# SHI-Labs/Self-Similarity-Grouping

Hardware: AMD Instinct MI355X
Metric: images/s embed + s/iter for NxN rerank+DBSCAN, N=16k, 1/2/4/8 GPU (higher is better)
Workload: dtype f32 (embed: split-half operands hi+lo on fp16 MFMA, fp32 accumulate, 6e-8 max error vs the fp32 reference features) / exact int64 via int8 MFMA digits + f64 + f16 (distance, re-rank: half semantics, bit-exact)

## Files before the change

### include/ssg_hip.h

```cpp
#ifndef SSG_HIP_H
#define SSG_HIP_H

#include <stddef.h>
#include <stdint.h>

#ifdef __cplusplus
extern "C" {
#endif

typedef struct ihipStream_t* ssg_stream_t;

#define SSG_OK 0
#define SSG_ERR_INVALID (-1)
#define SSG_ERR_HIP (-2)
#define SSG_ERR_OVERFLOW (-3)
#define SSG_ERR_NAN (-4)

const char* ssg_last_error(void);
int ssg_version(void);
uint16_t ssg_double_to_half_bits(double d);

int ssg_range_stats_f32(const float* a, int rows_a, const float* b, int rows_b, int d, float* out4, ssg_stream_t stream);
int ssg_row_norms_f64(const float* x, int n, int d, int round_to_half, double* norms, ssg_stream_t stream);
int ssg_sqdist_self_f16(const float* x, const double* norms, int N, int d, int row0, int nrows, int memory_save, uint16_t* D, uint32_t* rowmax,
// ... 106 lines not shown
int ssg_conv1x1_dual_nhwc_x(const void* in, const void* in2, const void* w, const float* bias, void* out, int B, int H, int W, int Cin,
                            int H2, int W2, int Cin2, int stride2, int Cout, int relu, int flags, float acc_scale, const float* ch_scale,
                            int32_t* overflow, ssg_stream_t stream);
#define SSG_CONV_W_TILED 4
int ssg_conv_weights_tile_supported(int Cout, int Kpad);
int ssg_conv_weights_tile(const void* w, int Cout, int Kpad, void* wt, ssg_stream_t stream);
int ssg_conv2d_nhwc_xt(const void* in, const void* w, const void* wt, const float* bias, const void* res, void* out, int B, int H, int W, int Cin,
                       int Cout, int KH, int KW, int stride, int pad, int relu, int flags, float acc_scale, const float* ch_scale,
                       int32_t* overflow, ssg_stream_t stream);
int ssg_conv1x1_dual_nhwc_xt(const void* in, const void* in2, const void* w, const void* wt, const float* bias, void* out, int B, int H, int W, int Cin,
                             int H2, int W2, int Cin2, int stride2, int Cout, int relu, int flags, float acc_scale, const float* ch_scale,
                             int32_t* overflow, ssg_stream_t stream);
int ssg_conv_pair_supported(int K1, int C, int N2);
int ssg_conv_pair_nhwc_x(const void* y2, const void* w3, const float* b3, const float* cs3, const void* res, void* out,
                         const void* w1n, const float* b1n, const float* cs1n, void* y1n, int M, int K1, int C, int N2,
                         int32_t* overflow, ssg_stream_t stream);
int ssg_bottleneck_supported(int H, int W, int CIN, int C, int MID);
int ssg_bottleneck_nhwc_x(const void* x, const void* w1, const float* b1, const float* cs1, const void* w2, const float* b2, const float* cs2,
                          const void* w3, const float* b3, const float* cs3, void* out, int B, int H, int W, int C, int MID,
                          int32_t* overflow, ssg_stream_t stream);
int ssg_bottleneck_ds_nhwc_x(const void* x, const void* w1, const float* b1, const float* cs1, const void* w2, const float* b2, const float* cs2,
                             const void* w3cat, const float* b3, const float* cs3, void* out, int B, int H, int W, int CIN, int C, int MID,
                             int32_t* overflow, ssg_stream_t stream);
int ssg_basicblock_supported(int H, int W, int C);
int ssg_basicblock_nhwc_x(const void* x, const void* w1, const float* b1, const float* cs1, const void* w2, const float* b2, const float* cs2,
                          void* out, int B, int H, int W, int C, int32_t* overflow, ssg_stream_t stream);
int ssg_stem_pool_supported(int H, int W);
int ssg_stem_pool_nchw_x(const float* images, int flip, const void* w, const float* bias, const float* ch_scale, void* out, int B, int H, int W,
                         int32_t* overflow, ssg_stream_t stream);
int ssg_nchw_to_nhwc4_h4l4(const float* in, void* out, int B, int H, int W, int flip, ssg_stream_t stream);
int ssg_maxpool3x3s2_h8l8(const void* in, void* out, int B, int H, int W, int C, ssg_stream_t stream);
int ssg_gap_stripes_h8l8(const void* in, float* out, int B, int H, int W, int C, int num_split, ssg_stream_t stream);
int ssg_h8l8_encode(const float* in, void* out, int64_t n, float scale, ssg_stream_t stream);
int ssg_h8l8_decode(const void* in, float* out, int64_t n, float scale, ssg_stream_t stream);
int ssg_pairwise_sqdist_f32(const float* x, const float* y, int m, int n, int d, int self_form, float* ws, float* out, ssg_stream_t stream);
int ssg_nchw_to_nhwc4(const float* in, float* out, int B, int H, int W, int flip, ssg_stream_t stream);
int ssg_maxpool3x3s2_nhwc(const float* in, float* out, int B, int H, int W, int C, ssg_stream_t stream);
int ssg_gap_stripes(const float* in, float* out, int B, int H, int W, int C, int num_split, ssg_stream_t stream);
int ssg_flip_sum_l2norm(const float* a, const float* b, float* out, int rows, int C, ssg_stream_t stream);

int ssg_knn_sets(const uint16_t* D, const int32_t* rank, int N, int row0, int nrows, int K, int cap, int32_t* a_idx, uint16_t* a_val,
                 int32_t* a_nnz, int32_t* overflow, ssg_stream_t stream);
int ssg_set_jaccard_rows(const int32_t* a_idx, const int32_t* a_nnz, int capA, const int64_t* colptr, const int32_t* inv_row, int N, int row0,
                         int nrows, uint16_t one_minus_lambda_half, uint16_t* Jp, ssg_stream_t stream);

int ssg_seqdist_f64(const float* x, int m, const float* y, int n, int d, int take_sqrt, double* out, int64_t ld, ssg_stream_t stream);
// ... 192 lines not shown
```

### self-similarity-grouping_amd/csrc/bottleneck.hip

```cpp
#include "ssg_common.h"
#include <cstdlib>

#ifndef SSG_BN_NT_STORE
#define SSG_BN_NT_STORE 1
#endif
#ifndef SSG_BN_NT_RES
#define SSG_BN_NT_RES 1
#endif

namespace ssg {
namespace bneck {

typedef float v16f __attribute__((ext_vector_type(16)));
typedef unsigned int v4u __attribute__((ext_vector_type(4)));
typedef _Float16 v8h __attribute__((ext_vector_type(8)));
typedef float v4f __attribute__((ext_vector_type(4)));

struct Params {
  const float* x; float* out;
  const float* w1; const float* b1; const float* cs1;
  const float* w2; const float* b2; const float* cs2;
  const float* w3; const float* b3; const float* cs3;
  int B, H;
  int* overflow;
  unsigned long long* prof = nullptr;
};
#ifdef SSG_BN_PROF
#define SSG_BN_STAMP(I_) { if (p.prof && threadIdx.x == 0) p.prof[(size_t)blockIdx.x * 8 + (I_)] = __builtin_readcyclecounter(); }
#else
#define SSG_BN_STAMP(I_)
#endif

constexpr int cmax(int a, int b) { return a > b ? a : b; }

template <int C, int MID, int IW, int TH, int CIN = C, int NW = 4>
struct Cfg {
  static constexpr int HROWS = TH + 2, NPIX1 = HROWS * IW, NPIX = TH * IW;
  static constexpr int NTHR = NW * 64, RPP = NTHR / 4;
#ifndef SSG_BN_K1T
#define SSG_BN_K1T 32
#endif
#ifndef SSG_BN_K1T4
#define SSG_BN_K1T4 32
#endif
  static constexpr int K1T = NW == 8 ? SSG_BN_K1T : SSG_BN_K1T4, KS1 = K1T / 16, CPR1 = 4 * KS1, RPP1 = NTHR / CPR1;
  static constexpr int XROWS = (NPIX1 + RPP1 - 1) / RPP1 * RPP1;
  static constexpr int P1 = 80;
  static constexpr int P1T = K1T * 4 + 16;
// ... 25 lines not shown
  return (unsigned)__builtin_bit_cast(unsigned short, a) | ((unsigned)__builtin_bit_cast(unsigned short, b) << 16);
}
__device__ __forceinline__ void encode4(const float4 v, uint2& hi, uint2& lo) {
  const _Float16 h0 = (_Float16)v.x, h1 = (_Float16)v.y, h2 = (_Float16)v.z, h3 = (_Float16)v.w;
  hi = make_uint2(pack2(h0, h1), pack2(h2, h3));
  lo = make_uint2(pack2((_Float16)(v.x - (float)h0), (_Float16)(v.y - (float)h1)), pack2((_Float16)(v.z - (float)h2), (_Float16)(v.w - (float)h3)));
}
__device__ __forceinline__ unsigned hi_nonfinite_bits(const uint2 hi) {
  return ((hi.x & 0x7c007c00u) + 0x04000400u) | ((hi.y & 0x7c007c00u) + 0x04000400u);
}
__device__ __forceinline__ float hlo(unsigned u) { return (float)__builtin_bit_cast(_Float16, (unsigned short)(u & 0xffffu)); }
__device__ __forceinline__ float hhi(unsigned u) { return (float)__builtin_bit_cast(_Float16, (unsigned short)(u >> 16)); }
__device__ __forceinline__ float4 decode4(const uint2 hi, const uint2 lo) {
  return make_float4(hlo(hi.x) + hlo(lo.x), hhi(hi.x) + hhi(lo.x), hlo(hi.y) + hlo(lo.y), hhi(hi.y) + hhi(lo.y));
}
__device__ __forceinline__ float4 relu4(float4 v) {
  return make_float4(v.x > 0.f ? v.x : 0.f, v.y > 0.f ? v.y : 0.f, v.z > 0.f ? v.z : 0.f, v.w > 0.f ? v.w : 0.f);
}

__device__ __forceinline__ void bn_dma16(const __amdgpu_buffer_rsrc_t r, unsigned lds_addr, unsigned voff, int soff) {
  __builtin_amdgcn_raw_ptr_buffer_load_lds(r, (__attribute__((address_space(3))) void*)(uintptr_t)lds_addr, 16, voff, soff, 0, 0);
}

template <int C, int MID, int IW, int TH, int CIN, int NW>
__global__ __launch_bounds__(NW * 64, NW == 4 ? 2 : 1) void bottleneck_kernel(Params p) {
  using K = Cfg<C, MID, IW, TH, CIN, NW>;
  constexpr bool DS = K::DS;
  extern __shared__ __attribute__((aligned(16))) unsigned char smem[];
  const int tid = (int)threadIdx.x, lane = tid & 63, wave = tid >> 6, l32 = lane & 31, h = lane >> 5;
  const int tiles_img = p.H / TH, ntiles = p.B * tiles_img;
  int T;
  {
    const int b = (int)blockIdx.x, q = ntiles / 8, r = ntiles % 8, x = b % 8, s = b / 8;
    T = (x < r ? x * (q + 1) : r * (q + 1) + (x - r) * q) + s;
  }
  const int img = T / tiles_img, ty0 = (T - img * tiles_img) * TH;
  SSG_BN_STAMP(0)
  if (K::ZERO_EARLY && tid < K::PY / 16) *reinterpret_cast<uint4*>(smem + K::ZERO_OFF + tid * 16) = make_uint4(0u, 0u, 0u, 0u);

  constexpr int RPP = K::RPP, RPP1 = K::RPP1, AU = K::XROWS / RPP1, WU = MID / RPP1;
  const int ck = tid & 3, r0 = tid >> 2;
  const int ck1 = tid % K::CPR1, r1 = tid / K::CPR1;
  const float* ximg = p.x + (int64_t)img * p.H * IW * CIN;
  const __amdgpu_buffer_rsrc_t xrsrc = __builtin_amdgcn_make_buffer_rsrc(const_cast<float*>(ximg), 0, (unsigned)(p.H * IW * CIN * 4), 0x00020000);
  constexpr int MT1 = K::NPIX1 / 32, NT1 = MID / 32;
  constexpr int WC1 = NT1 < NW / 2 ? NT1 : NW / 2, WR1 = NW / WC1, MTW1 = (MT1 + WR1 - 1) / WR1, NTW1 = NT1 / WC1;
  static_assert(NT1 % WC1 == 0 && (WR1 * MTW1) * 32 <= K::XROWS, "phase-1 tiles divide over the waves");
// ... 177 lines not shown
        v = relu4(v);
        if (!inside) v = make_float4(0.f, 0.f, 0.f, 0.f);
        uint2 hi, lo;
        encode4(v, hi, lo);
        ovf |= hi_nonfinite_bits(hi);
        unsigned char* d = smem + (hp0 + l32) * K::PY + (ch >> 3) * 32 + h * 8;
        *reinterpret_cast<uint2*>(d) = hi; *reinterpret_cast<uint2*>(d + 16) = lo;
      }
  }
  if (!K::ZERO_EARLY && tid < K::PY / 16) *reinterpret_cast<uint4*>(smem + K::ZERO_OFF + tid * 16) = make_uint4(0u, 0u, 0u, 0u);
  SSG_BN_STORE2(0, 0)
  __syncthreads();
  SSG_BN_STAMP(2)

  constexpr int WC2 = NW / 4, NT2 = MID / 32 / WC2;
  const int pt2 = wave / WC2, cb2 = (wave % WC2) * NT2;
  v16f acc2[NT2];
#pragma unroll
  for (int j = 0; j < NT2; j++)
#pragma unroll
    for (int r = 0; r < 16; r++) acc2[j][r] = 0.f;
  const int m2 = pt2 * 32 + l32, ty2 = m2 / IW, tx2 = m2 - ty2 * IW;
  float4 cs2r[NT2][4], b2r[NT2][4];
#pragma unroll
  for (int j = 0; j < NT2; j++)
#pragma unroll
    for (int q = 0; q < 4; q++) {
      cs2r[j][q] = *reinterpret_cast<const float4*>(p.cs2 + (cb2 + j) * 32 + 8 * q + 4 * h); b2r[j][q] = *reinterpret_cast<const float4*>(p.b2 + (cb2 + j) * 32 + 8 * q + 4 * h);
    }
#define SSG_BN_STEP2(KT_, S_, B_)                                                                                     \
  {                                                                                                                  \
    if ((KT_) + K::PD2 < K::NK2) SSG_BN_LOAD2((KT_) + K::PD2, S_)                                                     \
    _Pragma("unroll") for (int sub = 0; sub < K::KT2; sub++) {                                                       \
      const int kt_ = (KT_) * K::KT2 + sub;                                                                          \
      const int chunk = kt_ / 9, tap = kt_ - chunk * 9, r = tap / 3, s = tap - r * 3;                                \
      const int xin = tx2 + s - 1;                                                                                   \
      const int abase = (xin >= 0 && xin < IW) ? ((ty2 + r) * IW + xin) * K::PY : K::ZERO_OFF;                       \
      const unsigned char* wb = smem + K::W2_OFF + (B_) * K::BUF2 + (cb2 * 32 + l32) * K::P2 + sub * 128 + h * 32;     \
      v8h xh_[2], xl_[2], wh_[2][NT2], wl_[2][NT2];                                                                  \
      _Pragma("unroll") for (int ks = 0; ks < 2; ks++) {                                                             \
        const unsigned char* q_ = smem + abase + (chunk * 4 + ks * 2 + h) * 32;                                      \
        xh_[ks] = *reinterpret_cast<const v8h*>(q_); xl_[ks] = *reinterpret_cast<const v8h*>(q_ + 16);               \
        _Pragma("unroll") for (int j = 0; j < NT2; j++) {                                                            \
          wh_[ks][j] = *reinterpret_cast<const v8h*>(wb + j * 32 * K::P2 + ks * 64);                                 \
          wl_[ks][j] = *reinterpret_cast<const v8h*>(wb + j * 32 * K::P2 + ks * 64 + 16); }                          \
      }                                                                                                              \
      _Pragma("unroll") for (int ks = 0; ks < 2; ks++) {                                                             \
        _Pragma("unroll") for (int j = 0; j < NT2; j++) acc2[j] = __builtin_amdgcn_mfma_f32_32x32x16_f16(wh_[ks][j], xl_[ks], acc2[j], 0, 0, 0); \
        _Pragma("unroll") for (int j = 0; j < NT2; j++) acc2[j] = __builtin_amdgcn_mfma_f32_32x32x16_f16(wl_[ks][j], xh_[ks], acc2[j], 0, 0, 0); \
        _Pragma("unroll") for (int j = 0; j < NT2; j++) acc2[j] = __builtin_amdgcn_mfma_f32_32x32x16_f16(wh_[ks][j], xh_[ks], acc2[j], 0, 0, 0); \
      }                                                                                                              \
    }                                                                                                                \
    if ((KT_) + 1 < K::NK2) SSG_BN_STORE2((B_) ^ 1, ((S_) + 1) % K::PD2)                                              \
    __syncthreads();                                                                                                 \
  }
  static_assert(K::NK2 % 6 == 0 && 6 % K::PD2 == 0, "phase-2 ring");
#pragma unroll
  for (int kt0 = 0; kt0 < K::NK2; kt0 += 6) {
    SSG_BN_STEP2(kt0, 0 % K::PD2, 0) SSG_BN_STEP2(kt0 + 1, 1 % K::PD2, 1) SSG_BN_STEP2(kt0 + 2, 2 % K::PD2, 0)
    SSG_BN_STEP2(kt0 + 3, 3 % K::PD2, 1) SSG_BN_STEP2(kt0 + 4, 4 % K::PD2, 0) SSG_BN_STEP2(kt0 + 5, 5 % K::PD2, 1)
  }
#undef SSG_BN_STEP2
  SSG_BN_STAMP(3)
#undef SSG_BN_LOAD2
#undef SSG_BN_STORE2

  constexpr int CU3 = C / RPP;
  constexpr int K3 = MID + (DS ? CIN : 0);
  const float* w3p = p.w3 + (int64_t)r0 * K3 + ck * 4;
  v4f sc3[2][CU3];
#define SSG_BN_LOAD3(T_, S_)                                                                                         \
  { _Pragma("unroll") for (int u = 0; u < CU3; u++) sc3[S_][u] = *reinterpret_cast<const v4f*>(w3p + (int64_t)(RPP * u) * K3 + (T_) * 16); }
#define SSG_BN_STORE3(BUF_, S_)                                                                                      \
  { unsigned char* sb_ = smem + K::W3_OFF + (BUF_) * K::BUF3;                                                        \
    _Pragma("unroll") for (int u = 0; u < CU3; u++) *reinterpret_cast<v4f*>(sb_ + (r0 + RPP * u) * K::P1 + ck * 16) = sc3[S_][u]; }
  SSG_BN_LOAD3(0, 0)
  SSG_BN_LOAD3(1, 1)
  constexpr int WC3 = NW / 4, NT3 = C / 32 / WC3;
  const int pt3 = wave / WC3, cb3 = (wave % WC3) * NT3;
  const int64_t gpix0 = ((int64_t)img * p.H + ty0) * IW + pt3 * 32;
  constexpr int NXK = DS ? CIN / 16 : 1;
  v8h xrh[NXK], xrl[NXK];
  if constexpr (DS) {
    const float* xq = p.x + (gpix0 + l32) * CIN + h * 8;
#pragma unroll
    for (int t = 0; t < NXK; t++) { xrh[t] = *reinterpret_cast<const v8h*>(xq + t * 16); xrl[t] = *reinterpret_cast<const v8h*>(xq + t * 16 + 4); }
  }
  unsigned char* myrows = smem + (pt3 * 32) * K::PY;
#pragma unroll
// ... 108 lines not shown
      const float4 rw = rr[j & 1][it];
      float4 r4;
      {
        const unsigned a0 = __float_as_uint(rw.x), a1 = __float_as_uint(rw.y), a2 = __float_as_uint(rw.z), a3 = __float_as_uint(rw.w);
        const unsigned g0 = lane_xor1((odd ? a0 : a2)), g1 = lane_xor1((odd ? a1 : a3));
        const unsigned h0 = odd ? g0 : a0, h1 = odd ? g1 : a1, l0 = odd ? a2 : g0, l1 = odd ? a3 : g1;
        r4 = decode4(make_uint2(h0, h1), make_uint2(l0, l1));
      }
      v.x += r4.x; v.y += r4.y; v.z += r4.z; v.w += r4.w;
      }
      v = relu4(v);
      uint2 hp, lp;
      encode4(v, hp, lp);
      ovf |= hi_nonfinite_bits(hp);
      const unsigned rx = lane_xor1((odd ? hp.x : lp.x)), ry = lane_xor1((odd ? hp.y : lp.y));
      const uint4 stv = make_uint4(odd ? rx : hp.x, odd ? ry : hp.y, odd ? lp.x : rx, odd ? lp.y : ry);
#if SSG_BN_NT_STORE
      { const v4u sv_ = {stv.x, stv.y, stv.z, stv.w}; __builtin_nontemporal_store(sv_, reinterpret_cast<v4u*>(outp + (int64_t)pr * C + col)); }
#else
      *reinterpret_cast<uint4*>(outp + (int64_t)pr * C + col) = stv;
#endif
    }
    __builtin_amdgcn_fence(__ATOMIC_ACQ_REL, "wavefront");
  }
  if ((ovf & 0x80008000u) && p.overflow) *p.overflow = 1;
  SSG_BN_STAMP(5)
}

template <int C, int MID, int IW, int TH>
struct CfgH {
  static constexpr int NW = 4, NTHR = NW * 64, HROWS = TH + 2, NPIX1 = HROWS * IW, NPIX = TH * IW;
  static constexpr int MH = MID / 2;
  static constexpr int K1T = 32, P1T = K1T * 4, CPR1 = 8, RPP1 = NTHR / CPR1;
  static constexpr int XROWS = NPIX1, BUF1 = (XROWS + MID) * P1T;
  static constexpr int NK1 = C / K1T, PD1 = 2;
  static constexpr int PYH = MH * 4 + 16;
  static constexpr int ZERO_OFF = NPIX1 * PYH;
  static constexpr int P2 = 144, W2_OFF = (ZERO_OFF + PYH + 255) / 256 * 256, BUF2 = MID * P2;
  static constexpr int NK2H = (MH / 32) * 9, PD2 = 3;
  static constexpr int NCP = 128, NPASS = C / NCP, KT3 = MID / 32;
  static constexpr int EP = 36, PATCH = 32 * EP * 4;
  static constexpr int LDS = cmax(2 * BUF1, W2_OFF + 2 * BUF2);
  static_assert(NPIX == 128 && NPIX1 % RPP1 == 0 && MID % RPP1 == 0 && MH == 64 && MID == NCP && NK1 % PD1 == 0 && NK2H % 6 == 0 && KT3 == 4, "layer2 shape");
  static_assert(((NPIX1 + 31) / 32 + 1) / 2 == 3 && 6 * 32 <= XROWS + MID, "phase 1: 2 x 3 pixel tiles, the sixth one reads W1 rows of the stage");
  static_assert(RPP1 % 16 == 0 && XROWS % 16 == 0, "the swizzle of a row is that of its thread (r1) / its lane (l32)");
  static_assert(NW * PATCH <= ZERO_OFF && 32 * P2 == PATCH, "patches live in the dead y1 rows");
// ... 293 lines not shown
#else
        *reinterpret_cast<uint4*>(outp + (int64_t)pr * C + col) = stv;
#endif
      }
      __builtin_amdgcn_fence(__ATOMIC_ACQ_REL, "wavefront");
    }
  }
#undef SSG_BH_RESLOAD
#undef SSG_BH_STORE3
#undef SSG_BH_LOAD3
  if ((ovf & 0x80008000u) && p.overflow) *p.overflow = 1;
  SSG_BN_STAMP(5)
}

}
}

extern "C" int ssg_bottleneck_supported(int H, int W, int CIN, int C, int MID) {
  if (C == 256 && MID == 64 && (CIN == 256 || CIN == 64) && W == 32 && H > 0 && H % 4 == 0) return 1;
  if (C == 512 && MID == 128 && CIN == 512 && W == 16 && H > 0 && H % 8 == 0) return 1;
  return 0;
}

template <int C, int MID, int IW, int TH, int CIN, int NW>
static int launch_bottleneck(const ssg::bneck::Params& p, hipStream_t stream) {
  using namespace ssg::bneck;
  using K = Cfg<C, MID, IW, TH, CIN, NW>;
  static bool attr_set = false;
  if (!attr_set) {
    SSG_HIP(hipFuncSetAttribute((const void*)bottleneck_kernel<C, MID, IW, TH, CIN, NW>, hipFuncAttributeMaxDynamicSharedMemorySize, K::LDS));
    attr_set = true;
  }
  hipLaunchKernelGGL((bottleneck_kernel<C, MID, IW, TH, CIN, NW>), dim3(p.B * (p.H / TH)), dim3(NW * 64), K::LDS, stream, p);
  SSG_LAUNCH_CHECK("bottleneck_kernel");
  return SSG_OK;
}

template <int C, int MID, int IW, int TH>
static int launch_bottleneck_halves(const ssg::bneck::Params& p, hipStream_t stream) {
  using namespace ssg::bneck;
  using K = CfgH<C, MID, IW, TH>;
  static bool attr_set = false;
  if (!attr_set) {
    SSG_HIP(hipFuncSetAttribute((const void*)bottleneck_halves_kernel<C, MID, IW, TH>, hipFuncAttributeMaxDynamicSharedMemorySize, K::LDS));
    attr_set = true;
  }
  hipLaunchKernelGGL((bottleneck_halves_kernel<C, MID, IW, TH>), dim3(p.B * (p.H / TH)), dim3(K::NTHR), K::LDS, stream, p);
  SSG_LAUNCH_CHECK("bottleneck_halves_kernel");
  return SSG_OK;
}

#ifndef SSG_BN_L2_WAVES_DEFAULT
#define SSG_BN_L2_WAVES_DEFAULT 4
#endif

extern "C" int ssg_bottleneck_nhwc_x(const void* x, const void* w1, const float* b1, const float* cs1, const void* w2, const float* b2, const float* cs2,
                                     const void* w3, const float* b3, const float* cs3, void* out, int B, int H, int W, int C, int MID,
                                     int32_t* overflow, hipStream_t stream) {
  using namespace ssg::bneck;
  if (B <= 0 || !ssg_bottleneck_supported(H, W, C, C, MID) || !cs1 || !cs2 || !cs3 || x == out) {
    ssg_set_error("ssg_bottleneck_nhwc_x: unsupported block B=%d H=%d W=%d C=%d MID=%d (see ssg_bottleneck_supported)", B, H, W, C, MID);
    return SSG_ERR_INVALID;
  }
  Params p;
  p.x = (const float*)x; p.out = (float*)out;
  p.w1 = (const float*)w1; p.b1 = b1; p.cs1 = cs1; p.w2 = (const float*)w2; p.b2 = b2; p.cs2 = cs2; p.w3 = (const float*)w3; p.b3 = b3; p.cs3 = cs3;
  p.B = B; p.H = H; p.overflow = overflow;
  if (C == 512) {
    const char* e = getenv("SSG_BN_L2_WAVES");
    const int nw = e && *e ? atoi(e) : SSG_BN_L2_WAVES_DEFAULT;
    if (nw == 4) return launch_bottleneck_halves<512, 128, 16, 8>(p, stream);
    if (nw == 8) return launch_bottleneck<512, 128, 16, 8, 512, 8>(p, stream);
    ssg_set_error("ssg_bottleneck_nhwc_x: SSG_BN_L2_WAVES=%s (4 or 8)", e);
    return SSG_ERR_INVALID;
  }
  return launch_bottleneck<256, 64, 32, 4, 256, 4>(p, stream);
}

extern "C" int ssg_bottleneck_ds_nhwc_x(const void* x, const void* w1, const float* b1, const float* cs1, const void* w2, const float* b2, const float* cs2,
                                        const void* w3cat, const float* b3, const float* cs3, void* out, int B, int H, int W, int CIN, int C, int MID,
                                        int32_t* overflow, hipStream_t stream) {
  using namespace ssg::bneck;
  if (B <= 0 || CIN == C || !ssg_bottleneck_supported(H, W, CIN, C, MID) || !cs1 || !cs2 || !cs3) {
    ssg_set_error("ssg_bottleneck_ds_nhwc_x: unsupported block B=%d H=%d W=%d CIN=%d C=%d MID=%d (see ssg_bottleneck_supported)", B, H, W, CIN, C, MID);
    return SSG_ERR_INVALID;
  }
  Params p;
  p.x = (const float*)x; p.out = (float*)out;
  p.w1 = (const float*)w1; p.b1 = b1; p.cs1 = cs1; p.w2 = (const float*)w2; p.b2 = b2; p.cs2 = cs2; p.w3 = (const float*)w3cat; p.b3 = b3; p.cs3 = cs3;
  p.B = B; p.H = H; p.overflow = overflow;
// ... 3 lines not shown
```

### self-similarity-grouping_amd/resnet.py

```python
from collections import OrderedDict

import math
import os

import torch

from . import _lib
from ._lib import check, ptr, stream

_LAYERS = {18: (2, 2, 2, 2), 34: (3, 4, 6, 3), 50: (3, 4, 6, 3), 101: (3, 4, 23, 3), 152: (3, 8, 36, 3)}
_BASIC = (18, 34)
_BN_EPS = 1e-5
_DEC_CLUSTERS, _DEC_DIM, _DEC_KEY = 32, 2048, "assignment.cluster_centers"
_FUSED_BASICBLOCK_DEFAULT = "1"


def _expansion(depth):
    return 1 if depth in _BASIC else 4


def _arch(depth):
    blocks = []
    inplanes = 64
    exp = _expansion(depth)
# ... 39 lines not shown
        conv(p + ".conv1", pl, ip, 1); bn(p + ".bn1", pl)
        conv(p + ".conv2", pl, pl, 3); bn(p + ".bn2", pl)
        conv(p + ".conv3", pl * 4, pl, 1); bn(p + ".bn3", pl * 4)
        if blk["down"]:
            conv(p + ".downsample.0", pl * 4, ip, 1); bn(p + ".downsample.1", pl * 4)
    sd["base.fc.weight"] = torch.randn(1000, width, generator=g) * 0.01
    sd["base.fc.bias"] = torch.zeros(1000)
    if num_features > 0:
        sd["feat.weight"] = torch.randn(num_features, width, generator=g) * 0.001
        sd["feat_bn.weight"] = torch.ones(num_features); sd["feat_bn.bias"] = torch.zeros(num_features)
        sd["feat_bn.running_mean"] = torch.zeros(num_features); sd["feat_bn.running_var"] = torch.ones(num_features)
        sd["feat_bn.num_batches_tracked"] = torch.zeros((), dtype=torch.long)
    if cluster:
        bound = math.sqrt(6.0 / (_DEC_CLUSTERS + _DEC_DIM))
        sd[_DEC_KEY] = (torch.rand(_DEC_CLUSTERS, _DEC_DIM, generator=g) * 2.0 - 1.0) * bound
    return sd


class _FoldedConv:
    __slots__ = ("w", "bias", "cin", "cout", "k", "stride", "pad", "split", "acc_scale", "cscale", "wt")


_IN_SPLIT, _OUT_SPLIT, _W_TILED = 1, 2, 4


def _attach_tiled(f):
    f.wt = None
    cout, kp = f.w.shape
    if not f.split or f.cin == 4 or f.w.device.type != "cuda":
        return f
    L = _lib.lib()
    if not L.ssg_conv_weights_tile_supported(cout, kp):
        return f
    both = torch.empty((2, cout, kp), dtype=torch.float32, device=f.w.device)
    both[0].copy_(f.w)
    rc = L.ssg_conv_weights_tile(ptr(both[0]), cout, kp, ptr(both[1]), stream())
    if rc != 1:
        check(rc if rc < 0 else -2, "ssg_conv_weights_tile")
    f.w, f.wt = both[0], both[1]
    return f


def _h8l8(v):
    rows, K = v.shape
    hi = v.half()
    lo = (v - hi.float()).half()
# ... 258 lines not shown
                continue
            if blk["down"]:
                c3, ds = self._fold_dual(p, blk["stride"], sp)
            else:
                c3, ds = fold(p + ".conv3", p + ".bn3", 1, 0, sp), None
            net["blocks"].append(dict(
                c1=fold(p + ".conv1", p + ".bn1", 1, 0, sp),
                c2=fold(p + ".conv2", p + ".bn2", blk["stride"], 1, sp),
                c3=c3, ds=ds))
        self._folded = net
        return net

    @staticmethod
    def _conv(L, x, f, res=None, relu=True, out_split=False, ovf=None, tiled=False):
        B, H, W, _ = x.shape
        OH = (H + 2 * f.pad - f.k) // f.stride + 1; OW = (W + 2 * f.pad - f.k) // f.stride + 1
        out = torch.empty((B, OH, OW, f.cout), dtype=torch.float32, device=x.device)
        flags = (_IN_SPLIT if f.split else 0) | (_OUT_SPLIT if out_split else 0) | (_W_TILED if tiled and f.wt is not None else 0)
        check(L.ssg_conv2d_nhwc_x(ptr(x), ptr(f.w), ptr(f.bias), ptr(res), ptr(out), B, H, W, f.cin, f.cout, f.k, f.k, f.stride, f.pad,
                                  1 if relu else 0, flags, f.acc_scale, ptr(getattr(f, "cscale", None)), ptr(ovf), stream()), "ssg_conv2d_nhwc_x")
        return out

    @staticmethod
    def _conv_dual(L, o, x, c3, ds, out_split=False, ovf=None, tiled=False):
        B, H, W, _ = o.shape
        _, H2, W2, _ = x.shape
        out = torch.empty((B, H, W, c3.cout), dtype=torch.float32, device=o.device)
        flags = (_IN_SPLIT if ds.split else 0) | (_OUT_SPLIT if out_split else 0) | (_W_TILED if tiled and ds.wt is not None else 0)
        check(L.ssg_conv1x1_dual_nhwc_x(ptr(o), ptr(x), ptr(ds.w), ptr(ds.bias), ptr(out), B, H, W, c3.cin, H2, W2, ds.cin, ds.stride, c3.cout, 1,
                                        flags, ds.acc_scale, ptr(getattr(ds, "cscale", None)), ptr(ovf), stream()), "ssg_conv1x1_dual_nhwc_x")
        return out

    @staticmethod
    def _bottleneck(L, y, blk, ovf=None):
        B, H, W, CIN = y.shape
        c1, c2, c3, ds = blk["c1"], blk["c2"], blk["c3"], blk["ds"]
        if os.environ.get("SSG_FUSED_BOTTLENECK", "1") == "0" or c2.stride != 1 or (ds is not None and ds.stride != 1):
            return None
        if not L.ssg_bottleneck_supported(H, W, CIN, c3.cout, c1.cout):
            return None
        out = torch.empty((B, H, W, c3.cout), dtype=torch.float32, device=y.device)
        if ds is None:
            check(L.ssg_bottleneck_nhwc_x(ptr(y), ptr(c1.w), ptr(c1.bias), ptr(c1.cscale), ptr(c2.w), ptr(c2.bias), ptr(c2.cscale),
                                          ptr(c3.w), ptr(c3.bias), ptr(c3.cscale), ptr(out), B, H, W, CIN, c1.cout, ptr(ovf), stream()),
                  "ssg_bottleneck_nhwc_x")
        else:
            check(L.ssg_bottleneck_ds_nhwc_x(ptr(y), ptr(c1.w), ptr(c1.bias), ptr(c1.cscale), ptr(c2.w), ptr(c2.bias), ptr(c2.cscale),
                                             ptr(ds.w), ptr(ds.bias), ptr(ds.cscale), ptr(out), B, H, W, CIN, c3.cout, c1.cout, ptr(ovf), stream()),
                  "ssg_bottleneck_ds_nhwc_x")
        return out

    @staticmethod
    def _basicblock(L, y, blk, ovf=None):
        B, H, W, C = y.shape
        c1, c2 = blk["c1"], blk["c2"]
        if os.environ.get("SSG_FUSED_BASICBLOCK", _FUSED_BASICBLOCK_DEFAULT) == "0" or c1.stride != 1 or blk["ds"] is not None or c1.cout != C:
            return None
        if not L.ssg_basicblock_supported(H, W, C):
            return None
        out = torch.empty((B, H, W, C), dtype=torch.float32, device=y.device)
        check(L.ssg_basicblock_nhwc_x(ptr(y), ptr(c1.w), ptr(c1.bias), ptr(c1.cscale), ptr(c2.w), ptr(c2.bias), ptr(c2.cscale), ptr(out),
                                      B, H, W, C, ptr(ovf), stream()), "ssg_basicblock_nhwc_x")
        return out
# ... 8 lines not shown
        if C != 3:
            raise ValueError("expected RGB images [B,3,H,W]")
        ovf = self._overflow_flag() if sp else None
        if sp and os.environ.get("SSG_FUSED_STEM", "1") != "0" and L.ssg_stem_pool_supported(H, W):
            st = net["stem"]
            y = torch.empty((B, H // 4, W // 4, 64), dtype=torch.float32, device=self.device)
            check(L.ssg_stem_pool_nchw_x(ptr(x), 1 if flip else 0, ptr(st.w), ptr(st.bias), ptr(st.cscale), ptr(y), B, H, W, ptr(ovf), stream()),
                  "ssg_stem_pool_nchw_x")
        else:
            x4 = torch.empty((B, H, W, 4), dtype=torch.float32, device=self.device)
            if sp:
                check(L.ssg_nchw_to_nhwc4_h4l4(ptr(x), ptr(x4), B, H, W, 1 if flip else 0, stream()), "ssg_nchw_to_nhwc4_h4l4")
            else:
                check(L.ssg_nchw_to_nhwc4(ptr(x), ptr(x4), B, H, W, 1 if flip else 0, stream()), "ssg_nchw_to_nhwc4")
            y = self._conv(L, x4, net["stem"], out_split=sp, ovf=ovf)
            _, H2, W2, _ = y.shape
            p = torch.empty((B, (H2 + 1) // 2, (W2 + 1) // 2, 64), dtype=torch.float32, device=self.device)
            if sp:
                check(L.ssg_maxpool3x3s2_h8l8(ptr(y), ptr(p), B, H2, W2, 64, stream()), "ssg_maxpool3x3s2_h8l8")
            else:
                check(L.ssg_maxpool3x3s2_nhwc(ptr(y), ptr(p), B, H2, W2, 64, stream()), "ssg_maxpool3x3s2_nhwc")
            y = p
        pair = sp and os.environ.get("SSG_CONV_PAIR", "0") == "1"
        blocks, o1_next = net["blocks"], None
        for bi, blk in enumerate(blocks):
            if hooks and bi in hooks:
                hooks[bi]()
            if blk.get("kind") == "basic":
                fused = self._basicblock(L, y, blk, ovf) if sp else None
                if fused is not None:
                    y = fused
                    continue
                o = self._conv(L, y, blk["c1"], out_split=sp, ovf=ovf, tiled=tw)
                r = y if blk["ds"] is None else self._conv(L, y, blk["ds"], relu=False, out_split=sp, ovf=ovf, tiled=tw)
                y = self._conv(L, o, blk["c2"], res=r, relu=True, out_split=sp, ovf=ovf, tiled=tw)
                continue
            if sp:
                fused = self._bottleneck(L, y, blk, ovf)
                if fused is not None:
                    y = fused
                    continue
            o = o1_next if o1_next is not None else self._conv(L, y, blk["c1"], out_split=sp, ovf=ovf, tiled=tw)
            o1_next = None
            o = self._conv(L, o, blk["c2"], out_split=sp, ovf=ovf, tiled=tw)
            if blk["ds"] is not None:
                y = self._conv_dual(L, o, y, blk["c3"], blk["ds"], out_split=sp, ovf=ovf, tiled=tw)
                continue
            nxt = blocks[bi + 1]["c1"] if bi + 1 < len(blocks) else None
            Bo, Ho, Wo, _ = o.shape
            if (pair and nxt is not None and nxt.k == 1 and nxt.stride == 1 and nxt.cin == blk["c3"].cout and Bo * Ho * Wo >= 128 * 256
                    and L.ssg_conv_pair_supported(blk["c3"].cin, blk["c3"].cout, nxt.cout)):
                y, o1_next = self._conv_pair(L, o, blk["c3"], y, nxt, ovf)
            else:
                y = self._conv(L, o, blk["c3"], res=y, relu=True, out_split=sp, ovf=ovf, tiled=tw)
        return y, sp

    @staticmethod
    def _conv_pair(L, o, c3, res, c1n, ovf=None):
        B, H, W, _ = o.shape
        out = torch.empty((B, H, W, c3.cout), dtype=torch.float32, device=o.device)
        y1n = torch.empty((B, H, W, c1n.cout), dtype=torch.float32, device=o.device)
        check(L.ssg_conv_pair_nhwc_x(ptr(o), ptr(c3.w), ptr(c3.bias), ptr(c3.cscale), ptr(res), ptr(out), ptr(c1n.w), ptr(c1n.bias), ptr(c1n.cscale),
                                     ptr(y1n), B * H * W, c3.cin, c3.cout, c1n.cout, ptr(ovf), stream()), "ssg_conv_pair_nhwc_x")
        return out, y1n

    def _side_streams(self):
        st = getattr(self, "_streams", None)
        if st is None or st[0].device != self.device:
            prio = -1 if os.environ.get("SSG_FLIP_PRIO", "0") == "1" else 0
# ... 165 lines not shown
```

Baseline: 29090.

## Fuse next block's 1x1 conv and strided residual subsample into last layer1 bottleneck

Adds an NXT variant of the fused bottleneck kernel for the final layer1 identity block. The c3 epilogue feeds its output tile straight into the next block's c1 1x1 conv (MIDN=128) via MFMA and writes y1n. It also writes only a stride-2 subsampled copy of the block output for the downsample branch, skipping the full-resolution output write and the separate c1 conv launch and its reread. This adds LDS double-buffered weight streaming, a thread-local attach API and Python plumbing that passes stride 1 to the dual conv, at the cost of more register and LDS pressure inside the kernel.

```diff
diff --git a/include/ssg_hip.h b/include/ssg_hip.h
--- a/include/ssg_hip.h
+++ b/include/ssg_hip.h
@@ -152,6 +152,9 @@
 int ssg_bottleneck_ds_nhwc_x(const void* x, const void* w1, const float* b1, const float* cs1, const void* w2, const float* b2, const float* cs2,
                              const void* w3cat, const float* b3, const float* cs3, void* out, int B, int H, int W, int CIN, int C, int MID,
                              int32_t* overflow, ssg_stream_t stream);
+int ssg_bottleneck_next_supported(int H, int W, int C, int MID, int MIDN);
+int ssg_bottleneck_next_enabled(void);
+int ssg_bottleneck_attach_next(const void* w1n, const float* b1n, const float* cs1n, void* y1n, void* out_s2, int MIDN);
 int ssg_basicblock_supported(int H, int W, int C);
 int ssg_basicblock_nhwc_x(const void* x, const void* w1, const float* b1, const float* cs1, const void* w2, const float* b2, const float* cs2,
                           void* out, int B, int H, int W, int C, int32_t* overflow, ssg_stream_t stream);
diff --git a/self-similarity-grouping_amd/csrc/bottleneck.hip b/self-similarity-grouping_amd/csrc/bottleneck.hip
--- a/self-similarity-grouping_amd/csrc/bottleneck.hip
+++ b/self-similarity-grouping_amd/csrc/bottleneck.hip
@@ -24,6 +24,9 @@
   int B, H;
   int* overflow;
   unsigned long long* prof = nullptr;
+  const float* w1n = nullptr; const float* b1n = nullptr; const float* cs1n = nullptr;
+  float* y1n = nullptr;
+  float* out_s2 = nullptr;
 };
 #ifdef SSG_BN_PROF
 #define SSG_BN_STAMP(I_) { if (p.prof && threadIdx.x == 0) p.prof[(size_t)blockIdx.x * 8 + (I_)] = __builtin_readcyclecounter(); }
@@ -95,7 +98,7 @@
   __builtin_amdgcn_raw_ptr_buffer_load_lds(r, (__attribute__((address_space(3))) void*)(uintptr_t)lds_addr, 16, voff, soff, 0, 0);
 }
 
-template <int C, int MID, int IW, int TH, int CIN, int NW>
+template <int C, int MID, int IW, int TH, int CIN, int NW, bool NXT = false>
 __global__ __launch_bounds__(NW * 64, NW == 4 ? 2 : 1) void bottleneck_kernel(Params p) {
   using K = Cfg<C, MID, IW, TH, CIN, NW>;
   constexpr bool DS = K::DS;
@@ -319,6 +322,7 @@
     for (int r = 0; r < 16; r++) acc2[j][r] = 0.f;
   const int m2 = pt2 * 32 + l32, ty2 = m2 / IW, tx2 = m2 - ty2 * IW;
   float4 cs2r[NT2][4], b2r[NT2][4];
+  if constexpr (!NXT)
 #pragma unroll
   for (int j = 0; j < NT2; j++)
 #pragma unroll
@@ -362,6 +366,177 @@
 #undef SSG_BN_LOAD2
 #undef SSG_BN_STORE2
 
+  if constexpr (NXT) {
+  static_assert(!DS && NW == 4 && MID == 64 && C == 256 && IW == 32 && NT2 == 2 && WC2 == 1, "the layer1 identity block");
+  constexpr int MIDN = 128, NCP = 64, NPASS = C / NCP, NSTEP = 3 * NPASS;
+  constexpr int P3N = MID * 4 + 16, PN = 144, NXSTG = cmax(NCP * P3N, MIDN * PN);
+  constexpr int EP = 36, CPR = 8, RPI = 8, ITS = 4;
+  static_assert(K::W3_OFF + 2 * NXSTG <= K::LDS && 32 * EP * 4 <= 32 * K::PY && EP * 4 == PN && NPASS % 2 == 0, "ring behind the wave rows, patch in them");
+  const int ck16 = tid & 15, r16 = tid >> 4, ckn = tid & 7, rn = tid >> 3;
+  const __amdgpu_buffer_rsrc_t w3rsrc = __builtin_amdgcn_make_buffer_rsrc(const_cast<float*>(p.w3), 0, (unsigned)(C * MID * 4), 0x00020000);
+  const __amdgpu_buffer_rsrc_t wnrsrc = __builtin_amdgcn_make_buffer_rsrc(const_cast<float*>(p.w1n), 0, (unsigned)(MIDN * C * 4), 0x00020000);
+  const unsigned w3o = (unsigned)((r16 * MID + ck16 * 4) * 4), wno = (unsigned)((rn * C + ckn * 4) * 4);
+  v4f sn[2][4];
+#define SSG_BN_NLOAD(I_)                                                 \
+  { if (6 * pp + (I_) < NSTEP) { const int ps_ = 2 * pp + (I_) / 3;                                                  \
+      if constexpr ((I_) % 3 == 0) { _Pragma("unroll") for (int u = 0; u < 4; u++) sn[(I_) & 1][u] = __builtin_bit_cast(v4f, __builtin_amdgcn_raw_buffer_load_b128(w3rsrc, w3o, ((ps_ * NCP + 16 * u) * MID) * 4, 0)); } \
+      else { _Pragma("unroll") for (int u = 0; u < 4; u++) sn[(I_) & 1][u] = __builtin_bit_cast(v4f, __builtin_amdgcn_raw_buffer_load_b128(wnrsrc, wno, ((32 * u) * C + (2 * ps_ + (I_) % 3 - 1) * 32) * 4, 0)); } } }
+#define SSG_BN_NSTORE(I_)                                              \
+  { if (6 * pp + (I_) < NSTEP) { unsigned char* sb_ = smem + K::W3_OFF + ((I_) & 1) * NXSTG;                         \
+      if constexpr ((I_) % 3 == 0) { _Pragma("unroll") for (int u = 0; u < 4; u++) *reinterpret_cast<v4f*>(sb_ + (r16 + 16 * u) * P3N + ck16 * 16) = sn[(I_) & 1][u]; } \
+      else { _Pragma("unroll") for (int u = 0; u < 4; u++) *reinterpret_cast<v4f*>(sb_ + (rn + 32 * u) * PN + ckn * 16) = sn[(I_) & 1][u]; } } }
+  { constexpr int pp = 0; SSG_BN_NLOAD(0) SSG_BN_NLOAD(1) }
+  unsigned char* myrows = smem + (wave * 32) * K::PY;
+#pragma unroll
+  for (int j = 0; j < NT2; j++)
+#pragma unroll
+    for (int q = 0; q < 4; q++) {
+      const int ch = j * 32 + 8 * q + 4 * h;
+      const float4 cs = *reinterpret_cast<const float4*>(p.cs2 + ch), bi = *reinterpret_cast<const float4*>(p.b2 + ch);
+      float4 v = make_float4(acc2[j][4 * q] * cs.x + bi.x, acc2[j][4 * q + 1] * cs.y + bi.y, acc2[j][4 * q + 2] * cs.z + bi.z, acc2[j][4 * q + 3] * cs.w + bi.w);
+      v = relu4(v);
+      uint2 hi, lo;
+      encode4(v, hi, lo);
+      ovf |= hi_nonfinite_bits(hi);
+      unsigned char* d = myrows + l32 * K::PY + (ch >> 3) * 32 + h * 8;
+      *reinterpret_cast<uint2*>(d) = hi; *reinterpret_cast<uint2*>(d + 16) = lo;
+    }
+  __builtin_amdgcn_fence(__ATOMIC_ACQ_REL, "wavefront");
+  v8h y2h[MID / 16], y2l[MID / 16];
+#pragma unroll
+  for (int ks = 0; ks < MID / 16; ks++) {
+    const unsigned char* q_ = myrows + l32 * K::PY + (ks * 2 + h) * 32;
+    y2h[ks] = *reinterpret_cast<const v8h*>(q_); y2l[ks] = *reinterpret_cast<const v8h*>(q_ + 16);
+  }
+  __builtin_amdgcn_fence(__ATOMIC_ACQ_REL, "wavefront");
+  { constexpr int pp = 0; SSG_BN_NSTORE(0) }
+  __syncthreads();
+
+  const int chunk = lane % CPR, prow = lane / CPR, odd = lane & 1;
+  const int64_t gpix0 = ((int64_t)img * p.H + ty0) * IW + wave * 32;
+  const unsigned tpo = (unsigned)(((wave * 32 + prow) * C + chunk * 4) * 4);
+  const unsigned xro = (unsigned)(ty0 * IW * C * 4) + tpo;
+  const __amdgpu_buffer_rsrc_t orsrc = __builtin_amdgcn_make_buffer_rsrc(p.out ? p.out + ((int64_t)img * p.H + ty0) * IW * C : nullptr, 0,
+                                                                         p.out ? (unsigned)(K::NPIX * C * 4) : 0u, 0x00020000);
+  const __amdgpu_buffer_rsrc_t srsrc = __builtin_amdgcn_make_buffer_rsrc(p.out_s2 ? p.out_s2 + (((int64_t)img * (p.H / 2) + ty0 / 2) * (IW / 2)) * C : nullptr, 0,
+                                                                         p.out_s2 ? (unsigned)((TH / 2) * (IW / 2) * C * 4) : 0u, 0x00020000);
+  const unsigned s2o = ((wave | prow) & 1) ? 0x80000000u : (unsigned)((((wave >> 1) * (IW / 2) + (prow >> 1)) * C + chunk * 4) * 4);
+  float* const patch = reinterpret_cast<float*>(myrows);
+  const unsigned char* const patchb = myrows;
+  v16f acc3[NCP / 32], acc4[MIDN / 32];
+#pragma unroll
+  for (int j = 0; j < MIDN / 32; j++)
+#pragma unroll
+    for (int r = 0; r < 16; r++) acc4[j][r] = 0.f;
+  float4 rr[ITS], b3r, cs3r;
+  constexpr int NT_RES = SSG_BN_NT_RES ? 2 : 0, NT_ST = SSG_BN_NT_STORE ? 2 : 0;
+#define SSG_BN_NEPIOPS(T_)                                                                                           \
+  { _Pragma("unroll") for (int it = 0; it < ITS; it++) { const v4u t4_ = __builtin_amdgcn_raw_buffer_load_b128(xrsrc, xro, (it * RPI * C + (T_) * 32) * 4, NT_RES);  \
+      rr[it] = make_float4(__uint_as_float(t4_[0]), __uint_as_float(t4_[1]), __uint_as_float(t4_[2]), __uint_as_float(t4_[3])); } \
+    b3r = *reinterpret_cast<const float4*>(p.b3 + (T_) * 32 + chunk * 4); cs3r = *reinterpret_cast<const float4*>(p.cs3 + (T_) * 32 + chunk * 4); }
+  SSG_BN_NEPIOPS(0)
+#define SSG_BN_NSTEP3(I_)                                                                                            \
+  { SSG_BN_NLOAD((I_) + 2)                                                                                         \
+    _Pragma("unroll") for (int j = 0; j < NCP / 32; j++) _Pragma("unroll") for (int r = 0; r < 16; r++) acc3[j][r] = 0.f; \
+    const unsigned char* wb_ = smem + K::W3_OFF + ((I_) & 1) * NXSTG + l32 * P3N + h * 32;                            \
+    _Pragma("unroll") for (int ks = 0; ks < MID / 16; ks++) {                                                        \
+      const v8h xh_ = y2h[ks], xl_ = y2l[ks];                                                                        \
+      v8h wh_[NCP / 32], wl_[NCP / 32];                                                                              \
+      _Pragma("unroll") for (int j = 0; j < NCP / 32; j++) {                                                         \
+        wh_[j] = *reinterpret_cast<const v8h*>(wb_ + j * 32 * P3N + ks * 64); wl_[j] = *reinterpret_cast<const v8h*>(wb_ + j * 32 * P3N + ks * 64 + 16); } \
+      _Pragma("unroll") for (int j = 0; j < NCP / 32; j++) acc3[j] = __builtin_amdgcn_mfma_f32_32x32x16_f16(wh_[j], xl_, acc3[j], 0, 0, 0); \
+      _Pragma("unroll") for (int j = 0; j < NCP / 32; j++) acc3[j] = __builtin_amdgcn_mfma_f32_32x32x16_f16(wl_[j], xh_, acc3[j], 0, 0, 0); \
+      _Pragma("unroll") for (int j = 0; j < NCP / 32; j++) acc3[j] = __builtin_amdgcn_mfma_f32_32x32x16_f16(wh_[j], xh_, acc3[j], 0, 0, 0); \
+    }                                                                                                                \
+    SSG_BN_NSTORE((I_) + 1)                                                                                          \
+    __syncthreads();                                                                                                 \
+  }
+#define SSG_BN_NSTEPN(I_, J_)                                                                                        \
+  { const int ct_ = 2 * (2 * pp + (I_) / 3) + (J_);                                                                 \
+    SSG_BN_NLOAD((I_) + 2)                                                                                           \
+    const float4 bias = b3r, cs = cs3r;                                                                              \
+    _Pragma("unroll") for (int q = 0; q < 4; q++)                                                                    \
+      *reinterpret_cast<float4*>(patch + l32 * EP + 8 * q + 4 * h) = make_float4(acc3[J_][4 * q], acc3[J_][4 * q + 1], acc3[J_][4 * q + 2], acc3[J_][4 * q + 3]); \
+    __builtin_amdgcn_fence(__ATOMIC_ACQ_REL, "wavefront");                                                           \
+    _Pragma("unroll") for (int it = 0; it < ITS; it++) {                                                             \
+      const int pr = it * RPI + prow;                                                                                \
+      float4 v = *reinterpret_cast<const float4*>(patch + pr * EP + chunk * 4);                                      \
+      v.x = v.x * cs.x + bias.x; v.y = v.y * cs.y + bias.y; v.z = v.z * cs.z + bias.z; v.w = v.w * cs.w + bias.w;    \
+      const float4 rw = rr[it];                                                                                      \
+      float4 r4;                                                                                                     \
+      {    \
+        const unsigned a0 = __float_as_uint(rw.x), a1 = __float_as_uint(rw.y), a2 = __float_as_uint(rw.z), a3 = __float_as_uint(rw.w); \
+        const unsigned g0 = lane_xor1((odd ? a0 : a2)), g1 = lane_xor1((odd ? a1 : a3));                             \
+        const unsigned h0 = odd ? g0 : a0, h1 = odd ? g1 : a1, l0 = odd ? a2 : g0, l1 = odd ? a3 : g1;               \
+        r4 = decode4(make_uint2(h0, h1), make_uint2(l0, l1));                                                        \
+      }                                                                                                              \
+      v.x += r4.x; v.y += r4.y; v.z += r4.z; v.w += r4.w;                                                            \
+      v = relu4(v);                                                                                                  \
+      uint2 hp, lp;                                                                                                  \
+      encode4(v, hp, lp);                                                                                            \
+      ovf |= hi_nonfinite_bits(hp);                                                                                  \
+      const unsigned rx = lane_xor1((odd ? hp.x : lp.x)), ry = lane_xor1((odd ? hp.y : lp.y));                       \
+      const v4u sv_ = {odd ? rx : hp.x, odd ? ry : hp.y, odd ? lp.x : rx, odd ? lp.y : ry};                          \
+      *reinterpret_cast<v4u*>(patch + pr * EP + chunk * 4) = sv_;    \
+      if (p.out) __builtin_amdgcn_raw_buffer_store_b128(sv_, orsrc, tpo, (it * RPI * C + ct_ * 32) * 4, NT_ST);       \
+      if (p.out_s2) __builtin_amdgcn_raw_buffer_store_b128(sv_, srsrc, s2o, (it * (RPI / 2) * C + ct_ * 32) * 4, NT_ST); \
+    }                                                                                                                \
+    __builtin_amdgcn_fence(__ATOMIC_ACQ_REL, "wavefront");                                                           \
+    if (ct_ + 1 < C / 32) SSG_BN_NEPIOPS(ct_ + 1)                                                                    \
+    const unsigned char* wb_ = smem + K::W3_OFF + ((I_) & 1) * NXSTG + l32 * PN + h * 32;                             \
+    _Pragma("unroll") for (int ks = 0; ks < 2; ks++) {                                                               \
+      const unsigned char* q_ = patchb + l32 * PN + (ks * 2 + h) * 32;                                               \
+      const v8h xh_ = *reinterpret_cast<const v8h*>(q_), xl_ = *reinterpret_cast<const v8h*>(q_ + 16);               \
+      _Pragma("unroll") for (int jj = 0; jj < MIDN / 32; jj += 2) {        \
+        v8h wh_[2], wl_[2];                                                                                          \
+        _Pragma("unroll") for (int j = 0; j < 2; j++) {                                                              \
+          wh_[j] = *reinterpret_cast<const v8h*>(wb_ + (jj + j) * 32 * PN + ks * 64); wl_[j] = *reinterpret_cast<const v8h*>(wb_ + (jj + j) * 32 * PN + ks * 64 + 16); } \
+        _Pragma("unroll") for (int j = 0; j < 2; j++) acc4[jj + j] = __builtin_amdgcn_mfma_f32_32x32x16_f16(wh_[j], xl_, acc4[jj + j], 0, 0, 0); \
+        _Pragma("unroll") for (int j = 0; j < 2; j++) acc4[jj + j] = __builtin_amdgcn_mfma_f32_32x32x16_f16(wl_[j], xh_, acc4[jj + j], 0, 0, 0); \
+        _Pragma("unroll") for (int j = 0; j < 2; j++) acc4[jj + j] = __builtin_amdgcn_mfma_f32_32x32x16_f16(wh_[j], xh_, acc4[jj + j], 0, 0, 0); \
+      }                                                                                                              \
+    }                                                                                                                \
+    __builtin_amdgcn_fence(__ATOMIC_ACQ_REL, "wavefront");                                                           \
+    SSG_BN_NSTORE((I_) + 1)                                                                                          \
+    __syncthreads();                                                                                                 \
+  }
+#pragma unroll 1
+  for (int pp = 0; pp < NPASS / 2; pp++) {
+    SSG_BN_NSTEP3(0) SSG_BN_NSTEPN(1, 0) SSG_BN_NSTEPN(2, 1)
+    SSG_BN_NSTEP3(3) SSG_BN_NSTEPN(4, 0) SSG_BN_NSTEPN(5, 1)
+  }
+  SSG_BN_STAMP(4)
+#undef SSG_BN_NSTEPN
+#undef SSG_BN_NSTEP3
+#undef SSG_BN_NEPIOPS
+#undef SSG_BN_NSTORE
+#undef SSG_BN_NLOAD
+  if (p.y1n) {
+    float* __restrict__ ynp = p.y1n + gpix0 * MIDN;
+#pragma unroll
+    for (int j = 0; j < MIDN / 32; j++) {
+      const int col = j * 32 + chunk * 4;
+      const float4 bias = *reinterpret_cast<const float4*>(p.b1n + col), cs = *reinterpret_cast<const float4*>(p.cs1n + col);
+#pragma unroll
+      for (int q = 0; q < 4; q++)
+        *reinterpret_cast<float4*>(patch + l32 * EP + 8 * q + 4 * h) = make_float4(acc4[j][4 * q], acc4[j][4 * q + 1], acc4[j][4 * q + 2], acc4[j][4 * q + 3]);
+      __builtin_amdgcn_fence(__ATOMIC_ACQ_REL, "wavefront");
+#pragma unroll
+      for (int it = 0; it < ITS; it++) {
+        const int pr = it * RPI + prow;
+        float4 v = *reinterpret_cast<const float4*>(patch + pr * EP + chunk * 4);
+        v.x = v.x * cs.x + bias.x; v.y = v.y * cs.y + bias.y; v.z = v.z * cs.z + bias.z; v.w = v.w * cs.w + bias.w;
+        v = relu4(v);
+        uint2 hp, lp;
+        encode4(v, hp, lp);
+        ovf |= hi_nonfinite_bits(hp);
+        const unsigned rx = lane_xor1((odd ? hp.x : lp.x)), ry = lane_xor1((odd ? hp.y : lp.y));
+        *reinterpret_cast<uint4*>(ynp + (int64_t)pr * MIDN + col) = make_uint4(odd ? rx : hp.x, odd ? ry : hp.y, odd ? lp.x : rx, odd ? lp.y : ry);
+      }
+      __builtin_amdgcn_fence(__ATOMIC_ACQ_REL, "wavefront");
+    }
+  }
+  } else {
   constexpr int CU3 = C / RPP;
   constexpr int K3 = MID + (DS ? CIN : 0);
   const float* w3p = p.w3 + (int64_t)r0 * K3 + ck * 4;
@@ -516,6 +691,7 @@
 #endif
     }
     __builtin_amdgcn_fence(__ATOMIC_ACQ_REL, "wavefront");
+  }
   }
   if ((ovf & 0x80008000u) && p.overflow) *p.overflow = 1;
   SSG_BN_STAMP(5)
@@ -855,16 +1031,16 @@
   return 0;
 }
 
-template <int C, int MID, int IW, int TH, int CIN, int NW>
+template <int C, int MID, int IW, int TH, int CIN, int NW, bool NXT = false>
 static int launch_bottleneck(const ssg::bneck::Params& p, hipStream_t stream) {
   using namespace ssg::bneck;
   using K = Cfg<C, MID, IW, TH, CIN, NW>;
   static bool attr_set = false;
   if (!attr_set) {
-    SSG_HIP(hipFuncSetAttribute((const void*)bottleneck_kernel<C, MID, IW, TH, CIN, NW>, hipFuncAttributeMaxDynamicSharedMemorySize, K::LDS));
+    SSG_HIP(hipFuncSetAttribute((const void*)bottleneck_kernel<C, MID, IW, TH, CIN, NW, NXT>, hipFuncAttributeMaxDynamicSharedMemorySize, K::LDS));
     attr_set = true;
   }
-  hipLaunchKernelGGL((bottleneck_kernel<C, MID, IW, TH, CIN, NW>), dim3(p.B * (p.H / TH)), dim3(NW * 64), K::LDS, stream, p);
+  hipLaunchKernelGGL((bottleneck_kernel<C, MID, IW, TH, CIN, NW, NXT>), dim3(p.B * (p.H / TH)), dim3(NW * 64), K::LDS, stream, p);
   SSG_LAUNCH_CHECK("bottleneck_kernel");
   return SSG_OK;
 }
@@ -887,18 +1063,60 @@
 #define SSG_BN_L2_WAVES_DEFAULT 4
 #endif
 
+#ifndef SSG_BN_L1_NEXT_DEFAULT
+#define SSG_BN_L1_NEXT_DEFAULT 1
+#endif
+
+namespace {
+struct NextDesc { const float* w1n; const float* b1n; const float* cs1n; float* y1n; float* out_s2; int midn; bool set; };
+thread_local NextDesc g_next = {};
+}
+
+extern "C" int ssg_bottleneck_next_supported(int H, int W, int C, int MID, int MIDN) {
+  return (H > 0 && H % 4 == 0 && W == 32 && C == 256 && MID == 64 && MIDN == 128) ? 1 : 0;
+}
+
+extern "C" int ssg_bottleneck_next_enabled(void) {
+  const char* e = getenv("SSG_BN_L1_NEXT");
+  if (!e || !*e) return SSG_BN_L1_NEXT_DEFAULT;
+  if ((e[0] == '0' || e[0] == '1') && !e[1]) return e[0] - '0';
+  ssg_set_error("SSG_BN_L1_NEXT=%s (0 or 1)", e);
+  return SSG_ERR_INVALID;
+}
+
+extern "C" int ssg_bottleneck_attach_next(const void* w1n, const float* b1n, const float* cs1n, void* y1n, void* out_s2, int MIDN) {
+  g_next = NextDesc{};
+  if (!w1n || !b1n || !cs1n || MIDN != 128 || (y1n && y1n == out_s2)) {
+    ssg_set_error("ssg_bottleneck_attach_next: needs w1n, b1n, cs1n, MIDN = 128 and distinct outputs (MIDN=%d)", MIDN);
+    return SSG_ERR_INVALID;
+  }
+  g_next = NextDesc{(const float*)w1n, b1n, cs1n, (float*)y1n, (float*)out_s2, MIDN, true};
+  return SSG_OK;
+}
+
 extern "C" int ssg_bottleneck_nhwc_x(const void* x, const void* w1, const float* b1, const float* cs1, const void* w2, const float* b2, const float* cs2,
                                      const void* w3, const float* b3, const float* cs3, void* out, int B, int H, int W, int C, int MID,
                                      int32_t* overflow, hipStream_t stream) {
   using namespace ssg::bneck;
+  const NextDesc nd = g_next;
+  g_next = NextDesc{};
   if (B <= 0 || !ssg_bottleneck_supported(H, W, C, C, MID) || !cs1 || !cs2 || !cs3 || x == out) {
     ssg_set_error("ssg_bottleneck_nhwc_x: unsupported block B=%d H=%d W=%d C=%d MID=%d (see ssg_bottleneck_supported)", B, H, W, C, MID);
+    return SSG_ERR_INVALID;
+  }
+  if (nd.set && (!ssg_bottleneck_next_supported(H, W, C, MID, nd.midn) || x == nd.y1n || x == nd.out_s2 || (out && (out == nd.y1n || out == nd.out_s2)))) {
+    ssg_set_error("ssg_bottleneck_nhwc_x: no next-conv instance for B=%d H=%d W=%d C=%d MID=%d MIDN=%d with distinct tensors (see ssg_bottleneck_next_supported)",
+                  B, H, W, C, MID, nd.midn);
     return SSG_ERR_INVALID;
   }
   Params p;
   p.x = (const float*)x; p.out = (float*)out;
   p.w1 = (const float*)w1; p.b1 = b1; p.cs1 = cs1; p.w2 = (const float*)w2; p.b2 = b2; p.cs2 = cs2; p.w3 = (const float*)w3; p.b3 = b3; p.cs3 = cs3;
   p.B = B; p.H = H; p.overflow = overflow;
+  if (nd.set) {
+    p.w1n = nd.w1n; p.b1n = nd.b1n; p.cs1n = nd.cs1n; p.y1n = nd.y1n; p.out_s2 = nd.out_s2;
+    return launch_bottleneck<256, 64, 32, 4, 256, 4, true>(p, stream);
+  }
   if (C == 512) {
     const char* e = getenv("SSG_BN_L2_WAVES");
     const int nw = e && *e ? atoi(e) : SSG_BN_L2_WAVES_DEFAULT;
diff --git a/self-similarity-grouping_amd/resnet.py b/self-similarity-grouping_amd/resnet.py
--- a/self-similarity-grouping_amd/resnet.py
+++ b/self-similarity-grouping_amd/resnet.py
@@ -85,6 +85,13 @@
 
 
 _IN_SPLIT, _OUT_SPLIT, _W_TILED = 1, 2, 4
+
+
+def _next_enabled(L):
+    en = L.ssg_bottleneck_next_enabled()
+    if en < 0:
+        check(en, "ssg_bottleneck_next_enabled")
+    return en == 1
 
 
 def _attach_tiled(f):
@@ -389,23 +396,36 @@
         return out
 
     @staticmethod
-    def _conv_dual(L, o, x, c3, ds, out_split=False, ovf=None, tiled=False):
+    def _conv_dual(L, o, x, c3, ds, out_split=False, ovf=None, tiled=False, stride2=None):
         B, H, W, _ = o.shape
         _, H2, W2, _ = x.shape
         out = torch.empty((B, H, W, c3.cout), dtype=torch.float32, device=o.device)
         flags = (_IN_SPLIT if ds.split else 0) | (_OUT_SPLIT if out_split else 0) | (_W_TILED if tiled and ds.wt is not None else 0)
-        check(L.ssg_conv1x1_dual_nhwc_x(ptr(o), ptr(x), ptr(ds.w), ptr(ds.bias), ptr(out), B, H, W, c3.cin, H2, W2, ds.cin, ds.stride, c3.cout, 1,
+        check(L.ssg_conv1x1_dual_nhwc_x(ptr(o), ptr(x), ptr(ds.w), ptr(ds.bias), ptr(out), B, H, W, c3.cin, H2, W2, ds.cin,
+                                        ds.stride if stride2 is None else stride2, c3.cout, 1,
                                         flags, ds.acc_scale, ptr(getattr(ds, "cscale", None)), ptr(ovf), stream()), "ssg_conv1x1_dual_nhwc_x")
         return out
 
     @staticmethod
-    def _bottleneck(L, y, blk, ovf=None):
+    def _bottleneck(L, y, blk, ovf=None, nxt=None):
         B, H, W, CIN = y.shape
         c1, c2, c3, ds = blk["c1"], blk["c2"], blk["c3"], blk["ds"]
         if os.environ.get("SSG_FUSED_BOTTLENECK", "1") == "0" or c2.stride != 1 or (ds is not None and ds.stride != 1):
             return None
         if not L.ssg_bottleneck_supported(H, W, CIN, c3.cout, c1.cout):
             return None
+        if ds is None and nxt is not None and nxt.get("kind") != "basic" and nxt["ds"] is not None:
+            n1, n2, nds = nxt["c1"], nxt["c2"], nxt["ds"]
+            if (n1.k == 1 and n1.stride == 1 and n1.split and n1.cscale is not None and n1.cin == c3.cout and n2.stride == 2 and nds.stride == 2
+                    and H % 2 == 0 and W % 2 == 0 and L.ssg_bottleneck_next_supported(H, W, c3.cout, c1.cout, n1.cout)
+                    and _next_enabled(L)):
+                y1n = torch.empty((B, H, W, n1.cout), dtype=torch.float32, device=y.device)
+                out_s2 = torch.empty((B, H // 2, W // 2, c3.cout), dtype=torch.float32, device=y.device)
+                check(L.ssg_bottleneck_attach_next(ptr(n1.w), ptr(n1.bias), ptr(n1.cscale), ptr(y1n), ptr(out_s2), n1.cout), "ssg_bottleneck_attach_next")
+                check(L.ssg_bottleneck_nhwc_x(ptr(y), ptr(c1.w), ptr(c1.bias), ptr(c1.cscale), ptr(c2.w), ptr(c2.bias), ptr(c2.cscale),
+                                              ptr(c3.w), ptr(c3.bias), ptr(c3.cscale), None, B, H, W, CIN, c1.cout, ptr(ovf), stream()),
+                      "ssg_bottleneck_nhwc_x")
+                return y1n, out_s2
         out = torch.empty((B, H, W, c3.cout), dtype=torch.float32, device=y.device)
         if ds is None:
             check(L.ssg_bottleneck_nhwc_x(ptr(y), ptr(c1.w), ptr(c1.bias), ptr(c1.cscale), ptr(c2.w), ptr(c2.bias), ptr(c2.cscale),
@@ -460,7 +480,7 @@
                 check(L.ssg_maxpool3x3s2_nhwc(ptr(y), ptr(p), B, H2, W2, 64, stream()), "ssg_maxpool3x3s2_nhwc")
             y = p
         pair = sp and os.environ.get("SSG_CONV_PAIR", "0") == "1"
-        blocks, o1_next = net["blocks"], None
+        blocks, o1_next, y_is_s2 = net["blocks"], None, False
         for bi, blk in enumerate(blocks):
             if hooks and bi in hooks:
                 hooks[bi]()
@@ -474,7 +494,10 @@
                 y = self._conv(L, o, blk["c2"], res=r, relu=True, out_split=sp, ovf=ovf, tiled=tw)
                 continue
             if sp:
-                fused = self._bottleneck(L, y, blk, ovf)
+                fused = self._bottleneck(L, y, blk, ovf, nxt=blocks[bi + 1] if bi + 1 < len(blocks) else None)
+                if isinstance(fused, tuple):
+                    (o1_next, y), y_is_s2 = fused, True
+                    continue
                 if fused is not None:
                     y = fused
                     continue
@@ -482,7 +505,8 @@
             o1_next = None
             o = self._conv(L, o, blk["c2"], out_split=sp, ovf=ovf, tiled=tw)
             if blk["ds"] is not None:
-                y = self._conv_dual(L, o, y, blk["c3"], blk["ds"], out_split=sp, ovf=ovf, tiled=tw)
+                y = self._conv_dual(L, o, y, blk["c3"], blk["ds"], out_split=sp, ovf=ovf, tiled=tw, stride2=1 if y_is_s2 else None)
+                y_is_s2 = False
                 continue
             nxt = blocks[bi + 1]["c1"] if bi + 1 < len(blocks) else None
             Bo, Ho, Wo, _ = o.shape
```

Result: faster. 29580 (median of 6 runs) (+1.7%).
